# jesusdpa1/ssqueeze_rs

Measured on AMD Instinct MI355X. Metric: TF-bins/sec (ssq_stft, n_fft=1024), higher is better.
Workload: dtype f32

## Files before the change

### ssqueeze_rs_amd/csrc/stft_fused.hip

```cpp
#include "stft_fused_kernel.h"

namespace ssq {

struct Hi1024 {
  static constexpr int N = 1024, L = 64, NF = 513, W = 16, F = 16, PITCH = F + 1, THREADS = W * 64;
  static constexpr int PLANE = NF * PITCH;
  static constexpr int TILE_BYTES = (((2 * PLANE + F) * 4 + 15) / 16) * 16;
  static constexpr int EXH_ELEMS = 64 * 9;
  static constexpr int EXH_BYTES = W * EXH_ELEMS * 8;
  static constexpr int TAB_BYTES = N * 8;
  static constexpr int LDS_BYTES = TILE_BYTES + EXH_BYTES + 2 * TAB_BYTES;
  static constexpr int FRAC = 30, EMIN = -90;
  static_assert(LDS_BYTES <= 160 * 1024, "LDS budget");
};

__device__ __forceinline__ void rows_transpose4(float& r0, float& r1, float& r2, float& r3) {
  auto a = __builtin_amdgcn_permlane32_swap(__float_as_uint(r0), __float_as_uint(r2), false, false);
  auto b = __builtin_amdgcn_permlane32_swap(__float_as_uint(r1), __float_as_uint(r3), false, false);
  auto c = __builtin_amdgcn_permlane16_swap(a[0], b[0], false, false);
  auto d = __builtin_amdgcn_permlane16_swap(a[1], b[1], false, false);
  r0 = __uint_as_float(c[0]);
  r1 = __uint_as_float(c[1]);
  r2 = __uint_as_float(d[0]);
  r3 = __uint_as_float(d[1]);
}

template <bool EDGE, bool LEB, bool WKDBG = false>
__global__ __launch_bounds__(1024, 1) void stft_tx1024_kernel(StftDev<float> p) {
  using H = Hi1024;
  constexpr int THREADS = H::THREADS;
  using T = float;
  constexpr int N = H::N, L = H::L, NF = H::NF, F = H::F, PITCH = H::PITCH;
  __shared__ __attribute__((aligned(16))) unsigned char smem[H::LDS_BYTES];
  int* tile_re = reinterpret_cast<int*>(smem);
  float* col_scale = reinterpret_cast<float*>(tile_re + 2 * H::PLANE);
  cpx<T>* exch_all = reinterpret_cast<cpx<T>*>(smem + H::TILE_BYTES);
  cpx<T>* win_lds = reinterpret_cast<cpx<T>*>(smem + H::TILE_BYTES + H::EXH_BYTES);
  cpx<T>* tw1 = win_lds + N;
  cpx<T>* tw2 = tw1 + 256;

  const int tid = threadIdx.x;
  const int t = tid & 63;
  const int fl = __builtin_amdgcn_readfirstlane(tid >> 6);
  cpx<T>* exch = exch_all + fl * H::EXH_ELEMS;

  for (int i = tid; i < N; i += THREADS) win_lds[i] = p.win2[i];
  if (tid < 256) tw1[tid] = p.tw[((tid & 15) * (tid >> 4) * 4) & (N - 1)];
  for (int i = tid; i < 768; i += THREADS) tw2[i] = p.tw[((i & 255) * ((i >> 8) + 1)) & (N - 1)];
  constexpr long long CELL0 = WKDBG ? 0LL : 0x80000000LL;
  for (int i = tid; i < H::PLANE; i += THREADS) reinterpret_cast<long long*>(tile_re)[i] = CELL0;
  __syncthreads();
  const unsigned bid = blockIdx.x;
  if ((long long)bid >= p.total_tiles) return;

  const long long n_sig = p.total_tiles / p.tiles_per_signal;
  long long sig = (long long)(bid / (unsigned)p.tiles_per_signal);
  int jt = (int)(bid % (unsigned)p.tiles_per_signal);
  auto tile_frame0 = [&](int j) { return ((j < p.ta_n) ? p.ta0 + j : p.tb0 + (j - p.ta_n)) * F; };
  auto load_frame = [&](long long sg, int frame0, T (&xv)[16]) {
    const int frame = frame0 + fl;
    const T* xs = sig_base(p, sg);
    const long long pos0 = (long long)frame * p.hop - p.pad_left + t;
    if constexpr (!EDGE) {
#pragma unroll
      for (int q = 0; q < 16; ++q) xv[q] = xs[pos0 + L * q];
    } else {
      const bool valid = frame < p.n_frames;
      const long long first = pos0 - t;
      if (__all(valid && first >= 0 && first + N <= p.n_signal)) {
#pragma unroll
        for (int q = 0; q < 16; ++q) xv[q] = xs[pos0 + L * q];
      } else {
#pragma unroll
        for (int q = 0; q < 16; ++q) xv[q] = load_padded_flat<false>(xs, pos0 + L * q, p.n_signal, p.padtype, valid);
      }
    }
  };
  T xn[16];
  load_frame(sig, tile_frame0(jt), xn);
  const cpx<T> twr_unused[3][16] = {};

  auto read_out = [&](long long rsig, int rframe0) {
    if constexpr (!EDGE && !WKDBG) {
      if ((p.n_frames & 1) == 0) {
        constexpr int RS2 = THREADS / (F / 2);
        const int fp = tid % (F / 2);
        const int k0 = tid / (F / 2);
        float4* __restrict__ og4 = reinterpret_cast<float4*>(p.out + rsig * (long long)NF * p.n_frames + rframe0 + 2 * fp +
                                                             (long long)k0 * p.n_frames);
        const long long gstep4 = (long long)RS2 * p.n_frames / 2;
        const T sc0 = col_scale[2 * fp], sc1 = col_scale[2 * fp + 1];
        long long* tc = reinterpret_cast<long long*>(tile_re) + k0 * PITCH + 2 * fp;
        auto sweep2 = [&](int j) {
          const long long c0 = tc[j * RS2 * PITCH], c1 = tc[j * RS2 * PITCH + 1];
          tc[j * RS2 * PITCH] = CELL0;
          tc[j * RS2 * PITCH + 1] = CELL0;
          const int r0 = (int)c0 ^ (int)0x80000000, r1 = (int)c1 ^ (int)0x80000000;
          const int i0 = (int)(c0 >> 32), i1 = (int)(c1 >> 32);
          const float4 val = make_float4((T)r0 * sc0, (T)i0 * sc0, (T)r1 * sc1, (T)i1 * sc1);
          typedef float vf4 __attribute__((ext_vector_type(4)));
          const vf4 nv = {val.x, val.y, val.z, val.w};
          __builtin_nontemporal_store(nv, reinterpret_cast<vf4*>(&og4[j * gstep4]));
        };
        constexpr int NFULL2 = NF / RS2;
#pragma unroll
        for (int j = 0; j < NFULL2; ++j) sweep2(j);
        if (k0 + NFULL2 * RS2 < NF) sweep2(NFULL2);
        return;
      }
    }
    constexpr int RSTEP = THREADS / F;
    const int f = tid % F;
    const int k0 = tid / F;
    cpx<T>* __restrict__ og = p.out + rsig * (long long)NF * p.n_frames + rframe0 + f + (long long)k0 * p.n_frames;
    const long long gstep = (long long)RSTEP * p.n_frames;
    const bool fvalid = EDGE ? (rframe0 + f < p.n_frames) : true;
    const T sc = col_scale[f];
    constexpr int NFULL = NF / RSTEP;
    long long* tc = reinterpret_cast<long long*>(tile_re) + k0 * PITCH + f;
    auto sweep = [&](int j) {
      const long long c = tc[j * RSTEP * PITCH];
      tc[j * RSTEP * PITCH] = CELL0;
      if constexpr (WKDBG) {
        if (fvalid) og[j * gstep] = cpx<T>{__int_as_float((int)c), __int_as_float((int)(c >> 32))};
        return;
      }
      const int ire = (int)c ^ (int)0x80000000;
      const int iim = (int)(c >> 32);
      if (fvalid) og[j * gstep] = cpx<T>{(T)ire * sc, (T)iim * sc};
    };
#pragma unroll
    for (int j = 0; j < NFULL; ++j) sweep(j);
    if (k0 + NFULL * RSTEP < NF) sweep(NFULL);
  };

  const int grid_n = (int)gridDim.x;
#pragma unroll 1
  while (true) {
    const int frame0 = tile_frame0(jt);
    const bool valid = EDGE ? (frame0 + fl < p.n_frames) : true;
    long long nsig = sig;
    int njt = jt + grid_n;
    while (njt >= p.tiles_per_signal) {
      njt -= p.tiles_per_signal;
      ++nsig;
    }
    const bool has_next = nsig < n_sig;
    cpx<T> v[16];
#pragma unroll
    for (int q = 0; q < 16; ++q) {
      const cpx<T> wq = win_lds[t + L * q];
      v[q] = {xn[q] * wq.x, xn[q] * wq.y};
    }

    fft_compute<T, 10, 0, false, false>(v, twr_unused, tw1, t);
    {
      cpx<T> nv[16];
      const int rbase = 9 * (t >> 4) + (t & 7);
#pragma unroll
      for (int ph = 0; ph < 2; ++ph) {
#pragma unroll
        for (int u = 0; u < 8; ++u) exch[9 * t + u] = v[8 * ph + u];
        frame_sync<false>();
        if (((t >> 3) & 1) == ph) {
#pragma unroll
          for (int q = 0; q < 16; ++q) nv[q] = exch[rbase + 36 * q];
        }
        frame_sync<false>();
      }
#pragma unroll
      for (int q = 0; q < 16; ++q) v[q] = nv[q];
    }
    if (has_next) load_frame(nsig, tile_frame0(njt), xn);
    fft_compute<T, 10, 1, false, false, true>(v, twr_unused, tw1, t);
    {
#pragma unroll
      for (int uh = 0; uh < 4; ++uh) {
        rows_transpose4(v[4 * uh + 0].x, v[4 * uh + 1].x, v[4 * uh + 2].x, v[4 * uh + 3].x);
        rows_transpose4(v[4 * uh + 0].y, v[4 * uh + 1].y, v[4 * uh + 2].y, v[4 * uh + 3].y);
      }
#define SSQ_SWAP(i, j)       \
  {                          \
    const cpx<T> t_ = v[i];  \
    v[i] = v[j];             \
    v[j] = t_;               \
  }
      SSQ_SWAP(1, 4) SSQ_SWAP(2, 8) SSQ_SWAP(3, 12) SSQ_SWAP(6, 9) SSQ_SWAP(7, 13) SSQ_SWAP(11, 14)
#undef SSQ_SWAP
    }
    fft_compute<T, 10, 2, false, false, true>(v, twr_unused, tw2 - 256, t);

    cpx<T> zp[9];
    {
      const int src = (L - t) & (L - 1);
      zp[8] = v[8];
      if (t == 0) {
#pragma unroll
        for (int j = 8; j < 15; ++j) v[j] = v[j + 1];
        v[15] = v[0];
      }
#pragma unroll
      for (int q = 0; q < 8; ++q) {
        zp[q].x = __shfl(v[15 - q].x, src);
        zp[q].y = __shfl(v[15 - q].y, src);
      }
      v[8] = zp[8];
    }

    {
      cpx<T> cv[9];
      int dstb[9];
      T wdbg[9];
      int kdbg[9];
      T l1 = 0.0f;
      constexpr int CELL = 8;
      const float lane_on = valid ? 1.0f : 0.0f;
      const float sfs0 = (float)t * p.sfs_step, sfs_q = (float)L * p.sfs_step;
      const int neg_last = -(p.n_freqs - 1);
      constexpr bool NYQ = !LEB;
      constexpr int NQ = NYQ ? 8 : 9;
#pragma unroll
      for (int q = 0; q < NQ; ++q) {
        const cpx<T> zk = v[q], zn = zp[q];
        const cpx<T> S = {zk.x + zn.x, zk.y - zn.y};
        const cpx<T> dS = {zk.y + zn.y, zn.x - zk.x};
        const float den = S.x * S.x + S.y * S.y;
        const float num = dS.y * S.x - dS.x * S.y;
        const float pd = num * __builtin_amdgcn_rcpf(den * p.two_pi_eff);
        const float d = (sfs0 + (float)q * sfs_q) - pd;
        const float w = fabsf(d);
        float m = fma_clamp01(den, p.keep_big, p.keep_bias) * fma_clamp01(d, 0.0f, 1.0f);
        if constexpr (LEB) m = leb_keep_f32(m, den, w, p.gamma2);
        if (EDGE) m *= lane_on;
        if (q == 8) m *= (t == 0) ? 1.0f : 0.0f;
        const cpx<T> c = LEB ? cpx<T>{p.leb_unit * m, 0.0f} : cpx<T>{S.x * m, S.y * m};
        cv[q] = c;
        int kneg = cvt_floor_i32(__builtin_fmaf(-w, p.inv_dw, 0.5f));
        kneg = kneg < neg_last ? neg_last : kneg;
        if constexpr (LEB) kneg = (w != w) ? 0 : kneg;
        dstb[q] = __mul24(kneg, -(PITCH * CELL)) + fl * CELL;
        l1 += fabsf(c.x) + fabsf(c.y);
        if constexpr (WKDBG) {
          wdbg[q] = w;
          kdbg[q] = (m != 0.0f) ? -kneg : -1;
        }
      }
      if constexpr (NYQ) {
        const cpx<T> zk = v[8];
        const float sx = zk.x + zk.x, sy = zk.y - zk.y, dsx = zk.y + zk.y;
        const float den = __builtin_fmaf(sx, sx, sy);
        const float num = __builtin_fmaf(0.0f, sx, 0.0f * dsx);
        const float pd = num * __builtin_amdgcn_rcpf(den * p.two_pi_eff);
        const float d = (sfs0 + 8.0f * sfs_q) - pd;
        const float w = fabsf(d);
        float m = fma_clamp01(den, p.keep_big, p.keep_bias) * fma_clamp01(d, 0.0f, 1.0f);
        if (EDGE) m *= lane_on;
        m *= (t == 0) ? 1.0f : 0.0f;
        cv[8] = cpx<T>{sx * m, 0.0f};
        int kneg = cvt_floor_i32(__builtin_fmaf(-w, p.inv_dw, 0.5f));
        kneg = kneg < neg_last ? neg_last : kneg;
        dstb[8] = __mul24(kneg, -(PITCH * CELL)) + fl * CELL;
        l1 += fabsf(cv[8].x) + fabsf(sy);
        if constexpr (WKDBG) {
          wdbg[8] = w;
          kdbg[8] = (m != 0.0f) ? -kneg : -1;
        }
      }
      const T tot = frame_allreduce<T, L, false>(l1, t, nullptr, t) * p.dw;
      T scale, inv_scale;
      column_scale<T, H::FRAC, H::EMIN>(tot, p.dw, scale, inv_scale);
      if (t == 0 && valid) col_scale[fl] = inv_scale;
      char* ptile = reinterpret_cast<char*>(tile_re);
      if constexpr (WKDBG) {
#pragma unroll
        for (int q = 0; q < 9; ++q) {
          if ((q < 8 || t == 0) && valid) {
            const unsigned lo = (unsigned)__float_as_int(wdbg[q]), hi = (unsigned)__float_as_int((float)kdbg[q]);
            reinterpret_cast<unsigned long long*>(ptile)[(t + L * q) * PITCH + fl] = ((unsigned long long)hi << 32) | lo;
          }
        }
      } else {
#pragma unroll
        for (int q = 0; q < 9; ++q) {
          const int ia = cvt_round_i32(cv[q].x * scale);
          const int ib = (LEB || q == 8) ? 0 : cvt_round_i32(cv[q].y * scale);
          if (q < 8 || t == 0) {
            if (LEB) {
              atomicAdd(reinterpret_cast<unsigned*>(ptile + dstb[q]), (unsigned)ia);
            } else {
              const unsigned hi = (unsigned)(ib + (ia >> 31));
              atomicAdd(reinterpret_cast<unsigned long long*>(ptile + dstb[q]),
                        ((unsigned long long)hi << 32) | (unsigned)ia);
            }
          }
        }
      }
    }
    __syncthreads();
    read_out(sig, frame0);
    __syncthreads();
    if (!has_next) break;
    sig = nsig;
    jt = njt;
  }
}

template <typename T>
bool fused_supported(int n_fft) {
  return n_fft >= 64 && n_fft <= 4096 && (n_fft & (n_fft - 1)) == 0;
}

template <typename T, int LOGN>
static FusedLaunchShape shape_one(const StftDev<T>& p0, int cu_count, long long batch) {
  using C = FusedCfg<T, LOGN>;
  FusedLaunchShape s;
  int per_cu = (160 * 1024) / C::LDS_BYTES;
  if (per_cu < 1) per_cu = 1;
  if (per_cu * C::W > 32) per_cu = 32 / C::W;
  bool tx1024 = false;
  if constexpr (sizeof(T) == 4 && LOGN == 10) tx1024 = (p0.out_kind == 0 || p0.out_kind == 3) && p0.n_eff == C::N;
  s.tx1024 = tx1024;
  const int TF = tx1024 ? Hi1024::F : C::F;
  s.tile_frames = TF;
  const long long span = (long long)TF * p0.hop;
  const int tps_all = (p0.n_frames + TF - 1) / TF;
  long long lo = (p0.pad_left + span - 1) / span;
  long long hi_num = p0.n_signal - C::N - (long long)(TF - 1) * p0.hop + p0.pad_left;
  long long hi = hi_num >= 0 ? hi_num / span + 1 : 0;
  const long long full = p0.n_frames / TF;
  if (hi > full) hi = full;
  if (lo > tps_all) lo = tps_all;
  if (hi < lo) hi = lo;
  const long long blocks_one_wave = (long long)cu_count * (tx1024 ? 1 : per_cu);
  bool single_launch = (long long)tps_all * batch <= 4 * blocks_one_wave;
  if (const char* e = std::getenv("SSQ_SINGLE_LAUNCH")) single_launch = std::atoi(e) != 0;
  for (int edge = single_launch ? 1 : 0; edge < 2; ++edge) {
    FusedLaunchShape::Launch l;
    l.edge = edge;
    if (single_launch) {
      l.ta0 = 0;
      l.ta_n = tps_all;
      l.tb0 = 0;
      l.tiles_per_signal = tps_all;
    } else if (!edge) {
      l.ta0 = (int)lo;
      l.ta_n = (int)(hi - lo);
      l.tb0 = 0;
      l.tiles_per_signal = l.ta_n;
    } else {
      l.ta0 = 0;
      l.ta_n = (int)lo;
      l.tb0 = (int)hi;
      l.tiles_per_signal = (int)lo + (tps_all - (int)hi);
    }
    l.total_tiles = (long long)l.tiles_per_signal * batch;
    if (l.total_tiles <= 0) continue;
    l.blocks = tx1024 ? (long long)cu_count : (long long)cu_count * per_cu;
    if (l.blocks > l.total_tiles) l.blocks = l.total_tiles;
    s.launch[s.n_launch++] = l;
  }
  return s;
}

template <typename T, int LOGN>
static hipError_t launch_one(const StftDev<T>& p0, int cu_count, long long batch, hipStream_t stream) {
  using C = FusedCfg<T, LOGN>;
  const FusedLaunchShape s = shape_one<T, LOGN>(p0, cu_count, batch);
  const bool tx1024 = s.tx1024;
  for (int i = 0; i < s.n_launch; ++i) {
    const FusedLaunchShape::Launch& l = s.launch[i];
    const int edge = l.edge;
    StftDev<T> p = p0;
    p.ta0 = l.ta0;
    p.ta_n = l.ta_n;
    p.tb0 = l.tb0;
    p.tiles_per_signal = l.tiles_per_signal;
    p.total_tiles = l.total_tiles;
    const dim3 g((unsigned)l.blocks), b(C::W * 64);
    if constexpr (sizeof(T) == 4 && LOGN == 10) {
      if (tx1024) {
        const dim3 gh((unsigned)l.blocks), bh(Hi1024::THREADS);
        if (p.out_kind == 3) {
          if (edge) hipLaunchKernelGGL((stft_tx1024_kernel<true, false, true>), gh, bh, 0, stream, p);
          else hipLaunchKernelGGL((stft_tx1024_kernel<false, false, true>), gh, bh, 0, stream, p);
        } else if (p.squeezing == 1) {
          if (edge) hipLaunchKernelGGL((stft_tx1024_kernel<true, true>), gh, bh, 0, stream, p);
          else hipLaunchKernelGGL((stft_tx1024_kernel<false, true>), gh, bh, 0, stream, p);
        } else {
          if (edge) hipLaunchKernelGGL((stft_tx1024_kernel<true, false>), gh, bh, 0, stream, p);
          else hipLaunchKernelGGL((stft_tx1024_kernel<false, false>), gh, bh, 0, stream, p);
        }
        const hipError_t eh = hipGetLastError();
        if (eh != hipSuccess) return eh;
        continue;
      }
    }
    if (p.out_kind == 0 && p.squeezing == 1) {
      if (edge) hipLaunchKernelGGL((stft_fused_kernel<T, LOGN, true, true, true>), g, b, 0, stream, p);
      else hipLaunchKernelGGL((stft_fused_kernel<T, LOGN, true, false, true>), g, b, 0, stream, p);
    } else if (p.out_kind == 0) {
      if (edge) hipLaunchKernelGGL((stft_fused_kernel<T, LOGN, true, true, false>), g, b, 0, stream, p);
      else hipLaunchKernelGGL((stft_fused_kernel<T, LOGN, true, false, false>), g, b, 0, stream, p);
    } else if (p.out_kind == 3) {
      if (edge) hipLaunchKernelGGL((stft_fused_kernel<T, LOGN, true, true, false, true>), g, b, 0, stream, p);
      else hipLaunchKernelGGL((stft_fused_kernel<T, LOGN, true, false, false, true>), g, b, 0, stream, p);
    } else {
      if (edge) hipLaunchKernelGGL((stft_fused_kernel<T, LOGN, false, true, false>), g, b, 0, stream, p);
      else hipLaunchKernelGGL((stft_fused_kernel<T, LOGN, false, false, false>), g, b, 0, stream, p);
    }
    const hipError_t e = hipGetLastError();
    if (e != hipSuccess) return e;
  }
  return hipSuccess;
}

template <typename T>
int fused_tile_frames(int n_fft) {
  return for_fused_len(n_fft, 0, [](auto L) { return (int)FusedCfg<T, decltype(L)::value>::F; });
}

template <typename T>
hipError_t launch_stft_fused(const StftDev<T>& p, int n_fft, int cu_count, long long batch, hipStream_t stream) {
  if (p.n_eff != n_fft) return launch_stft_anylen<T>(p, n_fft, cu_count, batch, stream);
  return for_fused_len(n_fft, hipErrorInvalidValue,
                       [&](auto L) { return launch_one<T, decltype(L)::value>(p, cu_count, batch, stream); });
}

template <typename T>
hipError_t fused_launch_shape(const StftDev<T>& p, int n_fft, int cu_count, long long batch, FusedLaunchShape& shape) {
  if (p.n_eff != n_fft) return anylen_launch_shape<T>(p, n_fft, cu_count, batch, shape);
  return for_fused_len(n_fft, hipErrorInvalidValue, [&](auto L) {
    shape = shape_one<T, decltype(L)::value>(p, cu_count, batch);
    return hipSuccess;
  });
}

template bool fused_supported<float>(int);
template bool fused_supported<double>(int);
template int fused_tile_frames<float>(int);
template int fused_tile_frames<double>(int);
template hipError_t launch_stft_fused<float>(const StftDev<float>&, int, int, long long, hipStream_t);
template hipError_t launch_stft_fused<double>(const StftDev<double>&, int, int, long long, hipStream_t);
template hipError_t fused_launch_shape<float>(const StftDev<float>&, int, int, long long, FusedLaunchShape&);
template hipError_t fused_launch_shape<double>(const StftDev<double>&, int, int, long long, FusedLaunchShape&);

}
```

Baseline: 300.1 billion.

## Repack window, twiddle and exchange LDS tables for paired 16-byte reads

Reorders the window, stage-1 and stage-2 twiddle tables and the per-wave exchange buffer in LDS so that each thread reads two complex values at once with a single float4 load. The twiddle multiplies and butterflies for FFT passes 1 and 2 are inlined with these paired loads, and the exchange transpose is remapped to a new padded block layout. The goal is fewer LDS instructions and fewer bank conflicts in the FFT stages, at the cost of more intricate index mapping that must stay consistent across store, load and table fill.

```diff
diff --git a/ssqueeze_rs_amd/csrc/stft_fused.hip b/ssqueeze_rs_amd/csrc/stft_fused.hip
--- a/ssqueeze_rs_amd/csrc/stft_fused.hip
+++ b/ssqueeze_rs_amd/csrc/stft_fused.hip
@@ -1,4 +1,5 @@
 #include "stft_fused_kernel.h"
+#include "tx1024_lds_layout.h"
 
 namespace ssq {
 
@@ -6,13 +7,22 @@
   static constexpr int N = 1024, L = 64, NF = 513, W = 16, F = 16, PITCH = F + 1, THREADS = W * 64;
   static constexpr int PLANE = NF * PITCH;
   static constexpr int TILE_BYTES = (((2 * PLANE + F) * 4 + 15) / 16) * 16;
-  static constexpr int EXH_ELEMS = 64 * 9;
+  static constexpr int EXH_ELEMS = tx1024::EXCH_ELEMS;
   static constexpr int EXH_BYTES = W * EXH_ELEMS * 8;
-  static constexpr int TAB_BYTES = N * 8;
-  static constexpr int LDS_BYTES = TILE_BYTES + EXH_BYTES + 2 * TAB_BYTES;
+  static constexpr int TAB_BYTES = tx1024::TAB_ELEMS * 8;
+  static constexpr int LDS_BYTES = TILE_BYTES + EXH_BYTES + TAB_BYTES;
   static constexpr int FRAC = 30, EMIN = -90;
   static_assert(LDS_BYTES <= 160 * 1024, "LDS budget");
+  static_assert(N == tx1024::N && NF == tx1024::NF && W == tx1024::W && F == tx1024::F && PITCH == tx1024::PITCH &&
+                    TILE_BYTES == tx1024::TILE_BYTES && LDS_BYTES == tx1024::LDS_BYTES,
+                "tx1024_lds_layout.h describes this kernel's image (and asserts the 16-byte alignment of its parts)");
 };
+
+__device__ __forceinline__ void lds_pair(const cpx<float>* q, cpx<float>& a, cpx<float>& b) {
+  const float4 w = *reinterpret_cast<const float4*>(q);
+  a = {w.x, w.y};
+  b = {w.z, w.w};
+}
 
 __device__ __forceinline__ void rows_transpose4(float& r0, float& r1, float& r2, float& r3) {
   auto a = __builtin_amdgcn_permlane32_swap(__float_as_uint(r0), __float_as_uint(r2), false, false);
@@ -36,17 +46,18 @@
   float* col_scale = reinterpret_cast<float*>(tile_re + 2 * H::PLANE);
   cpx<T>* exch_all = reinterpret_cast<cpx<T>*>(smem + H::TILE_BYTES);
   cpx<T>* win_lds = reinterpret_cast<cpx<T>*>(smem + H::TILE_BYTES + H::EXH_BYTES);
-  cpx<T>* tw1 = win_lds + N;
-  cpx<T>* tw2 = tw1 + 256;
+  namespace X = tx1024;
+  cpx<T>* tw1 = win_lds + X::WIN_ELEMS;
+  cpx<T>* tw2 = tw1 + X::TW1_ELEMS;
 
   const int tid = threadIdx.x;
   const int t = tid & 63;
   const int fl = __builtin_amdgcn_readfirstlane(tid >> 6);
   cpx<T>* exch = exch_all + fl * H::EXH_ELEMS;
 
-  for (int i = tid; i < N; i += THREADS) win_lds[i] = p.win2[i];
-  if (tid < 256) tw1[tid] = p.tw[((tid & 15) * (tid >> 4) * 4) & (N - 1)];
-  for (int i = tid; i < 768; i += THREADS) tw2[i] = p.tw[((i & 255) * ((i >> 8) + 1)) & (N - 1)];
+  for (int s = tid; s < X::WIN_ELEMS; s += THREADS) win_lds[s] = p.win2[X::win_elem(s)];
+  for (int s = tid; s < X::TW1_ELEMS; s += THREADS) tw1[s] = p.tw[(X::tw1_k(s) * X::tw1_m(s) * 4) & (N - 1)];
+  for (int s = tid; s < X::TW2_ELEMS; s += THREADS) tw2[s] = p.tw[(X::tw2_j(s) * X::tw2_m(s)) & (N - 1)];
   constexpr long long CELL0 = WKDBG ? 0LL : 0x80000000LL;
   for (int i = tid; i < H::PLANE; i += THREADS) reinterpret_cast<long long*>(tile_re)[i] = CELL0;
   __syncthreads();
@@ -148,23 +159,25 @@
     const bool has_next = nsig < n_sig;
     cpx<T> v[16];
 #pragma unroll
-    for (int q = 0; q < 16; ++q) {
-      const cpx<T> wq = win_lds[t + L * q];
-      v[q] = {xn[q] * wq.x, xn[q] * wq.y};
-    }
-
-    fft_compute<T, 10, 0, false, false>(v, twr_unused, tw1, t);
+    for (int j = 0; j < 8; ++j) {
+      cpx<T> w0, w1;
+      lds_pair(win_lds + X::win_row(t, j), w0, w1);
+      v[2 * j] = {xn[2 * j] * w0.x, xn[2 * j] * w0.y};
+      v[2 * j + 1] = {xn[2 * j + 1] * w1.x, xn[2 * j + 1] * w1.y};
+    }
+
+    fft_compute<T, 10, 0, false, false>(v, twr_unused, nullptr, t);
     {
       cpx<T> nv[16];
-      const int rbase = 9 * (t >> 4) + (t & 7);
+      const int sbase = X::exch_store_base(t), lbase = X::exch_load_base(t);
 #pragma unroll
       for (int ph = 0; ph < 2; ++ph) {
 #pragma unroll
-        for (int u = 0; u < 8; ++u) exch[9 * t + u] = v[8 * ph + u];
+        for (int u = 0; u < 8; ++u) exch[sbase + X::exch_val(u)] = v[8 * ph + u];
         frame_sync<false>();
         if (((t >> 3) & 1) == ph) {
 #pragma unroll
-          for (int q = 0; q < 16; ++q) nv[q] = exch[rbase + 36 * q];
+          for (int g = 0; g < 8; ++g) lds_pair(exch + lbase + X::exch_load_off(g), nv[2 * g], nv[2 * g + 1]);
         }
         frame_sync<false>();
       }
@@ -172,7 +185,18 @@
       for (int q = 0; q < 16; ++q) v[q] = nv[q];
     }
     if (has_next) load_frame(nsig, tile_frame0(njt), xn);
-    fft_compute<T, 10, 1, false, false, true>(v, twr_unused, tw1, t);
+    {
+      const cpx<T>* row = tw1 + X::tw1_row(t & 15, 0);
+#pragma unroll
+      for (int i = 0; i < 8; ++i) {
+        cpx<T> w0, w1;
+        lds_pair(row + 2 * i, w0, w1);
+        v[2 * i + 1] = cmul(v[2 * i + 1], w0);
+        if (i < 7) v[2 * i + 2] = cmul(v[2 * i + 2], w1);
+      }
+      constexpr int R = pass_radix(10, 1), NB = 16 / R;
+      butterflies<false, R, NB>(v, std::make_integer_sequence<int, NB>{});
+    }
     {
 #pragma unroll
       for (int uh = 0; uh < 4; ++uh) {
@@ -188,7 +212,19 @@
       SSQ_SWAP(1, 4) SSQ_SWAP(2, 8) SSQ_SWAP(3, 12) SSQ_SWAP(6, 9) SSQ_SWAP(7, 13) SSQ_SWAP(11, 14)
 #undef SSQ_SWAP
     }
-    fft_compute<T, 10, 2, false, false, true>(v, twr_unused, tw2 - 256, t);
+    {
+      constexpr int R = pass_radix(10, 2), NB = 16 / R;
+      static_assert(R == 4 && NB == 4, "tw2 rows hold (b, m), b < 4, m = 1..3");
+#pragma unroll
+      for (int i = 0; i < 6; ++i) {
+        cpx<T> w0, w1;
+        lds_pair(tw2 + X::tw2_row(t, i), w0, w1);
+        const int e0 = 2 * i, e1 = 2 * i + 1;
+        v[e0 / 3 + (e0 % 3 + 1) * NB] = cmul(v[e0 / 3 + (e0 % 3 + 1) * NB], w0);
+        v[e1 / 3 + (e1 % 3 + 1) * NB] = cmul(v[e1 / 3 + (e1 % 3 + 1) * NB], w1);
+      }
+      butterflies<false, R, NB>(v, std::make_integer_sequence<int, NB>{});
+    }
 
     cpx<T> zp[9];
     {
diff --git a/ssqueeze_rs_amd/csrc/tx1024_lds_layout.h b/ssqueeze_rs_amd/csrc/tx1024_lds_layout.h
--- /dev/null
+++ b/ssqueeze_rs_amd/csrc/tx1024_lds_layout.h
@@ -0,0 +1,52 @@
+#pragma once
+
+namespace ssq {
+namespace tx1024 {
+
+constexpr int N = 1024, L = 64;
+
+constexpr int WIN_ELEMS = N;
+constexpr int win_row(int t, int j) { return 2 * (L * j + t); }
+constexpr int win_slot(int e) { return win_row(e & (L - 1), e >> 7) + ((e >> 6) & 1); }
+constexpr int win_elem(int s) { return ((s >> 1) & (L - 1)) + L * (2 * (s >> 7) + (s & 1)); }
+
+constexpr int TW1_PITCH = 18;
+constexpr int TW1_ELEMS = 16 * TW1_PITCH;
+constexpr int tw1_slot(int k, int m) { return TW1_PITCH * k + m - 1; }
+constexpr int tw1_row(int k, int i) { return tw1_slot(k, 2 * i + 1); }
+constexpr int tw1_k(int s) { return s / TW1_PITCH; }
+constexpr int tw1_m(int s) { return s % TW1_PITCH < 15 ? s % TW1_PITCH + 1 : 0; }
+
+constexpr int TW2_ELEMS = 3 * 256;
+constexpr int tw2_row(int t, int i) { return 2 * (L * i + t); }
+constexpr int tw2_slot(int t, int b, int m) { return tw2_row(t, (3 * b + m - 1) >> 1) + ((3 * b + m - 1) & 1); }
+constexpr int tw2_e(int s) { return 2 * (s >> 7) + (s & 1); }
+constexpr int tw2_j(int s) { return ((s >> 1) & (L - 1)) + L * (tw2_e(s) / 3); }
+constexpr int tw2_m(int s) { return tw2_e(s) % 3 + 1; }
+
+constexpr int TAB_ELEMS = WIN_ELEMS + TW1_ELEMS + TW2_ELEMS;
+
+constexpr int EXCH_ELEMS = 576;
+constexpr int exch_block(int r, int g) { return 66 * (2 * r + (g & 1)) + 16 * (g >> 1); }
+constexpr int exch_val(int u) { return 4 * (u & 3) + 2 * (u >> 2); }
+constexpr int exch_store_base(int a) { return exch_block(a & 3, a >> 3) + ((a >> 2) & 1); }
+constexpr int exch_load_base(int t) { return exch_block(t >> 4, 0) + exch_val(t & 7); }
+constexpr int exch_load_off(int g) { return exch_block(0, g); }
+constexpr int EXCH_USED = exch_block(3, 7) + 16;
+
+static_assert(EXCH_USED <= EXCH_ELEMS, "exchange row");
+static_assert(exch_block(3, 5) == exch_block(3, 0) + exch_load_off(5), "block index is additive in (r, g)");
+
+constexpr int NF = N / 2 + 1, F = 16, PITCH = F + 1, W = 16;
+constexpr int TILE_BYTES = (((2 * NF * PITCH + F) * 4 + 15) / 16) * 16;
+constexpr int EXCH_OFF = TILE_BYTES;
+constexpr int WIN_OFF = EXCH_OFF + W * EXCH_ELEMS * 8;
+constexpr int TW1_OFF = WIN_OFF + WIN_ELEMS * 8;
+constexpr int TW2_OFF = TW1_OFF + TW1_ELEMS * 8;
+constexpr int LDS_BYTES = TW2_OFF + TW2_ELEMS * 8;
+static_assert(EXCH_OFF % 16 == 0 && (EXCH_ELEMS * 8) % 16 == 0 && WIN_OFF % 16 == 0 && TW1_OFF % 16 == 0 && TW2_OFF % 16 == 0,
+              "16-byte reads: every table and every wave's exchange row starts 16-byte aligned");
+static_assert(LDS_BYTES <= 160 * 1024, "LDS budget");
+
+}
+}
```

New measurement: 309.6 billion (median of 6 runs). 1.03x the previous value.
